# tomneda/DABstar

Measured on AMD Instinct MI355X. Metric: DAB Mode-I ensembles/s (2.048 MS/s IQ->MSC bytes) per GPU; FIB CRC match %, higher is better.
Workload: dtype f32+i32

## Files before the change

### dabstar_amd/csrc/deliver.hip

```cpp
#include "pipeline.h"
#include "packet_core.h"
#include "pad_core.h"
#include "mot_core.h"
#include "carousel_core.h"
#include "mp2_core.h"
#include "aac_core.h"
#include "eti_core.h"
#include "tii_core.h"
#include "scope_core.h"
#include "fig00.h"

namespace dabx {

__global__ __launch_bounds__(128) void k_deliver_front(EngineDev e, DeliverDev dv)
{
  const int s = blockIdx.x, tid = threadIdx.x;
  const StreamCtl &c = e.ctl[s];
  uint8_t *slab = dv.slab;
  if (s == 0 && tid == 0) *reinterpret_cast<dabx_chunk_header *>(slab) = dv.hdr;
  const int F = dv.hdr.max_frames;
  const long long done = dv.frames_done[s], have = c.frames - done;
  int n = (int)(have < F ? have : F);
  if (n > e.out_frames) n = e.out_frames;
  if (!(dv.hdr.what & DABX_DELIVER_FIB)) n = (int)(have < F ? have : F);
// ... 39 lines not shown
  if (pre) {
    const BatchSnap bs = e.snap[sj / e.max_subch];
    cif_out += msc_new_frames(bs.msc_done, bs.cif_no, sc.start_cif).n;
  }
  const int cap_cifs = 4 * dv.hdr.max_frames;
  const long long have = cif_out - dv.cif_done[sj];
  LfRange q;
  q.n = (int)(have < cap_cifs ? have : cap_cifs);
  if (q.n > MSC_SLOTS) q.n = MSC_SLOTS;
  if (q.n < 0) q.n = 0;
  q.lost = (int)(have > q.n ? have - q.n : 0);
  q.first = cif_out - q.n;
  const bool want_lf = (dv.hdr.what & DABX_DELIVER_MSC) || ((dv.hdr.what & DABX_DELIVER_MSC_NOT_DABPLUS) && !sc.dab_plus);
  if (!want_lf) { q.lost = 0; q.first = cif_out; q.n = 0; }
  return q;
}

__global__ __launch_bounds__(64) void k_deliver_lf(EngineDev e, DeliverDev dv)
{
  const int sj = blockIdx.x, lane = threadIdx.x;
  const SubchDev &sc = e.subch[sj];
  if (!(sc.active && e.msc_out && !e.fic_only)) return;
  const LfRange q = deliver_lf_range(e, dv, sj, sc, true);
  if (q.n == 0) return;
  const uint8_t *ring = e.msc_out + (size_t)sj * MSC_SLOTS * e.msc_stride;
  uint32_t *o = reinterpret_cast<uint32_t *>(dv.slab + dv.layout_off[3 * (size_t)sj]);
  const int wpf = 3 * sc.kbps / 4;
  for (int f = 0; f < q.n; f++) {
    const uint32_t *src = reinterpret_cast<const uint32_t *>(ring + (size_t)((q.first + f) % MSC_SLOTS) * e.msc_stride);
    for (int w = lane; w < wpf; w += 64) o[(size_t)f * wpf + w] = src[w];
  }
}

__global__ __launch_bounds__(64) void k_deliver_msc(EngineDev e, DeliverDev dv, int with_lf)
{
  const int sj = blockIdx.x, lane = threadIdx.x;
  const SubchDev &sc = e.subch[sj];
  uint8_t *slab = dv.slab;
  const unsigned long long msc_off = dv.layout_off[3 * (size_t)sj], sf_off = dv.layout_off[3 * (size_t)sj + 1], sfi_off = dv.layout_off[3 * (size_t)sj + 2];
  const int R = sc.kbps / 8, nb = 3 * sc.kbps, sfb = 110 * R, pitch = (sfb + 3) & ~3;
  const int cap_sf = (4 * dv.hdr.max_frames + 4) / 5;
  long long c_done = dv.cif_done[sj], s_done = dv.sf_done[sj];
  int n_c = 0, n_s = 0, lost_c = 0, lost_s = 0;
  long long first_c = c_done, first_s = s_done;
  const bool live = sc.active && e.msc_out && !e.fic_only;
  if (live) {
    const long long have_s = sc.sf_count - s_done;
    const LfRange q = deliver_lf_range(e, dv, sj, sc, false);
    n_c = q.n; lost_c = q.lost; first_c = q.first;
    n_s = (int)(have_s < cap_sf ? have_s : cap_sf);
    if (n_s > SF_SLOTS) n_s = SF_SLOTS;
    if (n_s < 0) n_s = 0;
    lost_s = (int)(have_s > n_s ? have_s - n_s : 0);
    first_s = sc.sf_count - n_s;
    if (with_lf && n_c) {
      const uint8_t *ring = e.msc_out + (size_t)sj * MSC_SLOTS * e.msc_stride;
      uint32_t *o = reinterpret_cast<uint32_t *>(slab + msc_off);
      const int wpf = nb / 4;
      for (int f = 0; f < n_c; f++) {
        const uint32_t *src = reinterpret_cast<const uint32_t *>(ring + (size_t)((first_c + f) % MSC_SLOTS) * e.msc_stride);
        for (int w = lane; w < wpf; w += 64) o[(size_t)f * wpf + w] = src[w];
      }
    }
    if ((dv.hdr.what & DABX_DELIVER_SF) && sc.dab_plus) {
      const uint8_t *ring = e.sf_out + (size_t)sj * SF_SLOTS * e.sf_stride;
      uint32_t *o = reinterpret_cast<uint32_t *>(slab + sf_off);
      const int wpf = pitch / 4;
      for (int f = 0; f < n_s; f++) {
        const uint32_t *src = reinterpret_cast<const uint32_t *>(ring + (size_t)((first_s + f) % SF_SLOTS) * e.sf_stride);
        for (int w = lane; w < wpf; w += 64) o[(size_t)f * wpf + w] = src[w];
      }
      if (e.sf_info && lane < 8 * n_s) {
        const uint32_t *inf = reinterpret_cast<const uint32_t *>(e.sf_info + (size_t)sj * SF_SLOTS);
        uint32_t *oi = reinterpret_cast<uint32_t *>(slab + sfi_off);
        for (int w = lane; w < 8 * n_s; w += 64) oi[w] = inf[(size_t)((first_s + (w >> 3)) % SF_SLOTS) * 8 + (w & 7)];
      }
    }
  }
  if (lane == 0) {
    dabx_chunk_subch r;
    r.active = live ? 1 : 0; r.subch_id = dv.subch_id[sj]; r.kbps = sc.kbps; r.dab_plus = sc.dab_plus;
    r.start_cif = sc.start_cif; r.first_cif = first_c; r.n_cifs = n_c; r.cifs_lost = lost_c;
    r.first_sf = first_s; r.n_sf = n_s; r.sf_lost = lost_s; r.msc_off = msc_off; r.sf_off = sf_off; r.sf_pitch = pitch; r.reserved = 0;
    r.sf_ok = sc.sf_ok; r.sf_fail = sc.sf_fail; r.rs_corrected = sc.rs_corr; r.rs_failed = sc.rs_fail; r.fc_corrected = sc.fc_corr;
    r.au_ok = sc.au_ok; r.au_bad = sc.au_bad; r.sfi_off = sfi_off;
    reinterpret_cast<dabx_chunk_subch *>(slab + dv.hdr.off_subch)[sj] = r;
    if (live) { dv.cif_done[sj] = sc.cif_out; dv.sf_done[sj] = sc.sf_count; }
  }
}

__global__ __launch_bounds__(64) void k_deliver_dg(PacketDev pk, uint8_t *slab, unsigned long long off_dg)
{
  PacketSlot &ps = pk.slots[blockIdx.x];
  if (!ps.out.dl_rec_off) return;
  const OutGather g = out_ring_gather(ps.out, slab, threadIdx.x);
  if (threadIdx.x == 0) {
    dabx_chunk_dg t;
// ... 183 lines not shown
}

__global__ __launch_bounds__(256) void k_deliver_scope(EngineDev e, ScopeDeliverDev sd)
{
  const int s = blockIdx.x, tid = threadIdx.x;
  constexpr int CAP = DABX_CHUNK_FRAMES < SCOPE_RING ? DABX_CHUNK_FRAMES : SCOPE_RING, SLOT_Q = SCOPE_SLOT_BYTES / 16;
  static_assert(SCOPE_SLOT_BYTES % 16 == 0, "a record slot is copied in 16-byte words");
  const unsigned long long rec_off = sd.rec_off[s];
  const long long total = sd.ring ? sd.shows[(size_t)s * sd.st_stride] : 0, have = rec_off ? total - sd.done[s] : 0;
  int n = (int)(have < CAP ? have : CAP);
  if (n < 0) n = 0;
  const long long first = total - n;
  if (tid == 0) {
    dabx_chunk_scope r;
    r.first_record = first; r.n_records = n; r.records_lost = (int)(have > n ? have - n : 0); r.rec_off = rec_off; r.records_total = total;
    reinterpret_cast<dabx_chunk_scope *>(sd.slab + sd.off_scope)[s] = r;
  }
  uint4 *o = reinterpret_cast<uint4 *>(sd.slab + rec_off);
  for (int i = tid; i < n * SLOT_Q; i += 256) {
    const int k = i / SLOT_Q, wd = i - k * SLOT_Q;
    o[i] = reinterpret_cast<const uint4 *>(sd.ring + ((size_t)s * SCOPE_RING + (size_t)((first + k) % SCOPE_RING)) * SCOPE_SLOT_BYTES)[wd];
  }
  __syncthreads();
  if (tid == 0) sd.done[s] = total;
}

int launch_deliver_scope(const EngineDev &e, const ScopeDeliverDev &sd, hipStream_t st)
{
  hipLaunchKernelGGL(k_deliver_scope, dim3(e.n_streams), dim3(256), 0, st, e, sd);
  DABX_HIP(hipGetLastError());
  return 0;
}

int launch_deliver_msc(const EngineDev &e, const DeliverDev &dv, hipStream_t st, bool with_lf)
{
  if (e.max_subch <= 0) return 0;
  hipLaunchKernelGGL(k_deliver_msc, dim3(e.n_streams * e.max_subch), dim3(64), 0, st, e, dv, with_lf ? 1 : 0);
  DABX_HIP(hipGetLastError());
  return 0;
}
int launch_deliver_lf(const EngineDev &e, const DeliverDev &dv, hipStream_t st)
{
  if (e.max_subch <= 0 || !dv.lf_done) return 0;
  hipLaunchKernelGGL(k_deliver_lf, dim3(e.n_streams * e.max_subch), dim3(64), 0, st, e, dv);
  DABX_HIP(hipEventRecord(dv.lf_done, st));
  DABX_HIP(hipGetLastError());
  return 0;
}

__global__ __launch_bounds__(128) void k_eti_front(EngineDev e, EtiDev t)
{
  constexpr int F = MSC_BATCH_FRAMES;
  __shared__ int32_t found[12 * F], fhi[12 * F], flo[12 * F];
  const int s = blockIdx.x, tid = threadIdx.x;
  const StreamCtl &c = e.ctl[s];
  const EtiFront cur = t.front[s];
  EtiStage &st = t.stage[s];
  const long long frames = c.frames, have = frames - cur.fib_frames;
  const int n = have < 0 ? 0 : (int)(have < F ? have : F);
  const long long first = frames - n;
  for (int i = tid; i < n * 96; i += 128) {
    const int f = i / 96, w = i - 96 * f;
    const size_t slot = (size_t)s * e.out_frames + (size_t)((first + f) % e.out_frames);
    st.fib[f][w] = reinterpret_cast<const uint32_t *>(e.fib_out + slot * 384)[w];
  }
  for (int q = tid; q < 12 * n; q += 128) {
    const int f = q / 12, i = q - 12 * f;
    const size_t slot = (size_t)s * e.out_frames + (size_t)((first + f) % e.out_frames);
    int hi = -1, lo = -1;
    found[q] = e.fib_crc[slot * 12 + i] && fib_fig00_counter(e.fib_out + slot * 384 + 32 * i, &hi, &lo);
// ... 207 lines not shown
```

### dabstar_amd/csrc/engine.h

```cpp
#pragma once
#include "pipeline.h"
#include "packet_core.h"
#include "pad_core.h"
#include "mot_core.h"
#include "carousel_core.h"
#include "mp2_core.h"
#include "aac_core.h"
#include "tii_core.h"
#include "scope_core.h"
#include "sdma.h"
#include "iqfile.h"
#include <algorithm>
#include <condition_variable>
#include <deque>
#include <mutex>
#include <string>
#include <thread>
#include <vector>

using namespace dabx;

static constexpr int DL_FRAMES = MSC_BATCH_FRAMES;

struct Delivery {
  bool open = false;
  int what = 0;
  int copy_engine = 0;
  static constexpr int NDEV = 3;
  uint8_t *dev[NDEV] = {nullptr, nullptr, nullptr};
  hipEvent_t packed[NDEV] = {nullptr, nullptr, nullptr};
  hipEvent_t packed_lf[NDEV] = {nullptr, nullptr, nullptr};
  bool dev_busy[NDEV] = {false, false, false};
  hipStream_t cs = nullptr;
  Sdma sdma;
  size_t capacity = 0, bytes = 0;
  enum { FREE = 0, IN_FLIGHT = 1, LANDED = 2, HELD = 3 };
  struct Slot { uint8_t *host = nullptr; uint64_t sig = 0, sig2 = 0; int state = FREE; uint64_t seq = 0; size_t bytes = 0, lf_from = 0; int devslab = 0; };
  std::vector<Slot> slots;
  std::deque<int> queue;
  std::deque<int> jobs;
  std::mutex mu;
  std::condition_variable cv;
  std::thread copier;
  bool quit = false;
  int device = 0;
  std::string copier_error;
  uint64_t next_seq = 0, landed = 0, bytes_copied = 0;
  double copy_s = 0, copy_s_max = 0, gather_wait_s = 0, calib_gbps = 0;
  unsigned long long *layout_off = nullptr;
  int32_t *subch_id = nullptr;
  long long *frames_done = nullptr, *cif_done = nullptr, *sf_done = nullptr;
  dabx_chunk_header hdr{};
  bool want_pad = false;
  bool want_mot = false;
  bool want_dg = false;
  EtiFront *eti_front = nullptr;
  long long *eti_next = nullptr;
  EtiStage *eti_stage[NDEV] = {nullptr, nullptr, nullptr};
  size_t eti_rows_off = 0;
  dabx_chunk_header_ext ext{};
  long long *tii_done = nullptr;
  long long *scope_done = nullptr;
  unsigned long long *scope_off = nullptr;
  std::vector<char> scope_room;
  bool scope() const { return (what & DABX_DELIVER_SCOPE) != 0; }
  bool tii() const { return (what & DABX_DELIVER_TII) != 0; }
  bool mp2_audio() const { return (what & DABX_DELIVER_MP2_AUDIO) != 0; }
  bool aac() const { return (what & DABX_DELIVER_AAC) != 0; }
  bool eti() const { return (what & DABX_DELIVER_ETI) != 0; }
  EtiDev eti_dev(int devslab) const
  {
    return EtiDev{eti_front, eti_next, eti_stage[devslab], dev[devslab], subch_id, hdr.off_eti, eti_rows_off, hdr.max_frames, 0};
  }
};

struct Ingest {
  bool open = false;
  int copy_engine = 0, max_frames = 0;
  size_t capacity = 0;
  struct Slab {
    uint8_t *host = nullptr, *dev = nullptr; uint64_t sig = 0; bool in_flight = false;
    size_t bytes = 0, pitch = 0;
    std::vector<size_t> n_bytes;
    IqJob *jobs_host = nullptr, *jobs_dev = nullptr;
// ... 179 lines not shown
```

### dabstar_amd/csrc/engine_delivery.cpp

```cpp
#include "engine.h"
#include <algorithm>
#include <chrono>
#include <cstddef>
#include <cstring>
#include <string>
#include <thread>
#include <vector>

static_assert(sizeof(dabx_chunk_header) == 128 && sizeof(dabx_chunk_stream) == 72 && sizeof(dabx_chunk_frame) == 16 && sizeof(dabx_chunk_subch) == 144 && offsetof(dabx_chunk_header, off_mot) == 112 &&
              sizeof(dabx_superframe_info) == 32 && sizeof(dabx_chunk_eti) == 64 && offsetof(dabx_chunk_header, off_eti) == 120 &&
              sizeof(dabx_chunk_header_ext) == 64 && sizeof(dabx_chunk_tii) == 32 && sizeof(dabx_tii_event) == 32 && sizeof(dabx_tii_result) == 16 &&
              sizeof(dabx_chunk_mp2_audio) == 128 && offsetof(dabx_chunk_header_ext, off_mp2_audio) == 16 &&
              sizeof(dabx_chunk_aac) == 128 && offsetof(dabx_chunk_header_ext, off_aac) == 24,
              "include/dabx.h: chunk record layout");
static constexpr int DL_SF_CAP = (4 * DL_FRAMES + 4) / 5;
#if DABX_MSC_BATCH == 7
static_assert(DL_FRAMES == DABX_CHUNK_FRAMES, "include/dabx.h: DABX_CHUNK_FRAMES is the library's MSC batch");
#endif

template <class Tab> static size_t layout_section(Tab &tab, bool want, size_t off, size_t table_bytes, uint64_t *off_table)
{
  bool any = false;
  for (auto &q : tab.host) { q.st.out.dl_rec_off = q.st.out.dl_bytes_off = 0; any = any || q.on; }
  if (!want || !any) return off;
// ... 97 lines not shown

int dabx_engine::delivery_begin(DeliverDev *dv, int *slot, int *devslab)
{
  Delivery &D = dl;
  int h = -1;
  uint64_t seq;
  {
    std::unique_lock<std::mutex> lk(D.mu);
    if (!D.copier_error.empty()) { set_error("delivery: %s", D.copier_error.c_str()); return DABX_E_HIP; }
    for (size_t i = 0; i < D.slots.size() && h < 0; i++) if (D.slots[i].state == Delivery::FREE) h = (int)i;
    if (h < 0) { set_error("delivery: no free host slab (dabx_delivery_release)"); return DABX_E_STATE; }
    seq = D.next_seq++;
    const int k = (int)(seq % Delivery::NDEV);
    if (!D.cv.wait_for(lk, std::chrono::seconds(30), [&]() { return !D.dev_busy[k] || !D.copier_error.empty(); })) {
      D.next_seq--;
      set_error("delivery: device slab %d still busy after 30 s (chunk %llu)", k, (unsigned long long)seq);
      return DABX_E_STATE;
    }
    if (!D.copier_error.empty()) { D.next_seq--; set_error("delivery: %s", D.copier_error.c_str()); return DABX_E_HIP; }
    D.dev_busy[k] = true;
    D.slots[(size_t)h].state = Delivery::IN_FLIGHT;
    D.slots[(size_t)h].seq = seq;
    D.slots[(size_t)h].devslab = k;
    *devslab = k;
  }
  dv->slab = D.dev[*devslab]; dv->layout_off = D.layout_off; dv->subch_id = D.subch_id;
  dv->frames_done = D.frames_done; dv->cif_done = D.cif_done; dv->sf_done = D.sf_done;
  dv->hdr = D.hdr; dv->hdr.seq = seq;
  dv->off_mp2_audio = D.ext.off_mp2_audio;
  dv->off_aac = D.ext.off_aac;
  const size_t lf_from = (size_t)D.hdr.off_msc;
  const bool split = D.copy_engine == 0 && D.bytes > lf_from && D.bytes - lf_from >= ((size_t)1 << 20) && !dev.fic_only && dev.max_subch > 0 && dev.msc_out;
  dv->lf_done = split ? D.packed_lf[*devslab] : nullptr;
  {
    std::lock_guard<std::mutex> lk(D.mu);
    D.slots[(size_t)h].lf_from = split ? lf_from : 0;
  }
  *slot = h;
  int rc = launch_deliver_front(dev, *dv, stream);
  if (!rc && D.eti()) rc = launch_eti_front(dev, D.eti_dev(*devslab), stream, mk);
  if (!rc && D.tii())
    rc = launch_deliver_tii(dev, TiiDeliverDev{D.dev[*devslab], D.ext, D.tii_done, tiis.dev.ring, tiis.exists() ? &tiis.dev.cnt->events : nullptr,
                                               (int32_t)(sizeof(TiiCounters) / sizeof(long long)), 0}, stream);
  else if (!rc && D.ext.magic) rc = launch_deliver_ext(D.ext, D.dev[*devslab], stream);
  if (!rc && D.scope())
    rc = launch_deliver_scope(dev, ScopeDeliverDev{D.dev[*devslab], D.ext.off_scope, D.scope_off, D.scope_done, scope.dev.ring,
                                                   scope.exists() ? &scope.dev.st->shows : nullptr, (int32_t)(sizeof(ScopeState) / sizeof(long long)), 0}, stream);
  if (rc) {
    std::lock_guard<std::mutex> lk(D.mu);
    D.dev_busy[*devslab] = false;
    D.slots[(size_t)h].state = Delivery::FREE;
    D.next_seq--;
    D.cv.notify_all();
  }
  return rc;
}

void dabx_engine::delivery_abort(int slot, int devslab)
{
  Delivery &D = dl;
  std::lock_guard<std::mutex> lk(D.mu);
  D.slots[(size_t)slot].state = Delivery::FREE;
  D.dev_busy[devslab] = false;
  if (D.next_seq > 0) D.next_seq--;
  if (D.copier_error.empty()) D.copier_error = "a chunk was abandoned after a failed launch: " + std::string(dabx::last_error());
  D.cv.notify_all();
}

int dabx_engine::delivery_finish(int slot, int devslab, hipStream_t tail)
{
  Delivery &D = dl;
  {
    const hipError_t he = hipEventRecord(D.packed[devslab], tail);
    if (he != hipSuccess) {
      set_error("HIP error %d (%s) at %s:%d", (int)he, hipGetErrorString(he), __FILE__, __LINE__);
      delivery_abort(slot, devslab);
      return DABX_E_HIP;
    }
  }
  std::lock_guard<std::mutex> lk(D.mu);
  D.slots[(size_t)slot].bytes = D.bytes;
  D.queue.push_back(slot);
  D.jobs.push_back(slot);
  D.cv.notify_all();
  return 0;
// ... 65 lines not shown
  return 0;
}

void delivery_free(dabx_engine *e)
{
  Delivery &D = e->dl;
  if (D.copier.joinable()) {
    { std::lock_guard<std::mutex> lk(D.mu); D.quit = true; D.cv.notify_all(); }
    D.copier.join();
  }
  D.quit = false;
  if (D.cs) (void)hipStreamSynchronize(D.cs);
  for (auto &sl : D.slots) { if (sl.host) (void)hipHostFree(sl.host); sdma_signal_destroy(sl.sig); sdma_signal_destroy(sl.sig2); }
  D.slots.clear();
  D.queue.clear();
  D.jobs.clear();
  for (int k = 0; k < Delivery::NDEV; k++) {
    if (D.dev[k]) (void)hipFree(D.dev[k]);
    if (D.packed[k]) (void)hipEventDestroy(D.packed[k]);
    if (D.packed_lf[k]) (void)hipEventDestroy(D.packed_lf[k]);
    D.dev[k] = nullptr; D.packed[k] = nullptr; D.packed_lf[k] = nullptr; D.dev_busy[k] = false;
  }
  for (void *q : {(void *)D.layout_off, (void *)D.subch_id, (void *)D.frames_done, (void *)D.cif_done, (void *)D.sf_done, (void *)D.eti_front,
                  (void *)D.eti_next, (void *)D.eti_stage[0], (void *)D.eti_stage[1], (void *)D.eti_stage[2], (void *)D.tii_done, (void *)D.scope_done,
                  (void *)D.scope_off}) if (q) (void)hipFree(q);
  D.tii_done = nullptr; D.ext = dabx_chunk_header_ext{};
  D.scope_done = nullptr; D.scope_off = nullptr; D.scope_room.clear();
  D.layout_off = nullptr; D.subch_id = nullptr; D.frames_done = D.cif_done = D.sf_done = nullptr;
  D.eti_front = nullptr; D.eti_next = nullptr; D.eti_rows_off = 0;
  for (int k = 0; k < Delivery::NDEV; k++) D.eti_stage[k] = nullptr;
  if (D.cs) (void)hipStreamDestroy(D.cs);
  D.cs = nullptr;
  D.copier_error.clear();
  D.open = false; D.capacity = D.bytes = 0; D.next_seq = 0;
  D.landed = D.bytes_copied = 0; D.copy_s = D.copy_s_max = D.gather_wait_s = 0;
}

}

extern "C" {

int dabx_delivery_open(dabx_engine *e, const dabx_delivery_config *cfg)
{
  if (!e || (cfg && (cfg->host_slabs < 0 || cfg->host_slabs == 1 || cfg->host_slabs > 64 || (cfg->what & ~(1023 | DABX_DELIVER_AAC | DABX_DELIVER_SCOPE)) || cfg->copy_engine < 0 || cfg->copy_engine > 1))) {
    set_error("dabx_delivery_open: bad argument");
    return DABX_E_ARG;
  }
  if (cfg && cfg->what == DABX_DELIVER_TII) {
    set_error("dabx_delivery_open: DABX_DELIVER_TII needs at least one other DABX_DELIVER_* bit beside it");
    return DABX_E_ARG;
  }
  if (cfg && (cfg->what & DABX_DELIVER_MP2_AUDIO) && !(cfg->what & ~(DABX_DELIVER_MP2_AUDIO | DABX_DELIVER_TII))) {
    set_error("dabx_delivery_open: DABX_DELIVER_MP2_AUDIO needs at least one DABX_DELIVER_* bit below 256 beside it");
    return DABX_E_ARG;
  }
  if (cfg && (cfg->what & DABX_DELIVER_AAC) && !(cfg->what & ~(DABX_DELIVER_AAC | DABX_DELIVER_MP2_AUDIO | DABX_DELIVER_TII))) {
    set_error("dabx_delivery_open: DABX_DELIVER_AAC needs at least one DABX_DELIVER_* bit below 256 beside it");
    return DABX_E_ARG;
  }
  if (cfg && (cfg->what & DABX_DELIVER_SCOPE) &&
      !(cfg->what & ~(DABX_DELIVER_SCOPE | DABX_DELIVER_AAC | DABX_DELIVER_MP2_AUDIO | DABX_DELIVER_TII | DABX_DELIVER_ETI))) {
    set_error("dabx_delivery_open: DABX_DELIVER_SCOPE needs at least one DABX_DELIVER_* bit below 128 beside it");
    return DABX_E_ARG;
  }
  if (e->dl.open) { set_error("dabx_delivery_open: already open"); return DABX_E_STATE; }
  int rc = sync_all(e);
  if (rc) return rc;
// ... 193 lines not shown
```

### dabstar_amd/csrc/engine_facade.cpp

```cpp
#include "engine.h"
#include "viterbi_core.h"
#include <cstring>
#include <vector>

static int fic_engine_create(int batch, dabx_engine **out)
{
  auto *e = *out = new dabx_engine();
  (void)hipGetDevice(&e->device);
  if (hipStreamCreateWithFlags(&e->stream, hipStreamNonBlocking) != hipSuccess) { delete e; *out = nullptr; return DABX_E_HIP; }
  e->ss.a = e->stream;
  EngineDev &d = e->dev;
  d.n_streams = batch; d.max_subch = 0; d.out_frames = 1; d.fic_only = 1;
  d.vit_stride = (int)vit_scratch_words(FIC_OUT);
  int rc;
  if ((rc = e->alloc(&d.ctl, batch)) || (rc = e->alloc(&d.fic_sym, (size_t)batch * 3 * K2)) || (rc = e->alloc(&d.fib_out, (size_t)batch * 384)) ||
      (rc = e->alloc(&d.fib_crc, (size_t)batch * 12)) || (rc = e->alloc(&d.vit_scratch, (size_t)batch * 4 * d.vit_stride, false))) return rc;
  std::vector<StreamCtl> ctl(batch);
  for (auto &c : ctl) { memset(&c, 0, sizeof(c)); c.frame_ok = 1; }
  DABX_HIP(hipMemcpyAsync(d.ctl, ctl.data(), sizeof(StreamCtl) * batch, hipMemcpyHostToDevice, e->stream));
  DABX_HIP(hipStreamSynchronize(e->stream));
  return 0;
}

extern "C" {
// ... 422 lines not shown
  m->slots[(size_t)slot] = dabx_subch_desc{};
  return msc_apply(m);
}

int dabx_msc_stop_all_services(dabx_msc *m)
{
  if (!m) return DABX_E_ARG;
  for (auto &s : m->slots) s = dabx_subch_desc{};
  return msc_apply(m);
}

int dabx_msc_is_service_running(dabx_msc *m, int slot)
{
  if (!m || slot < 0 || slot >= (int)m->slots.size()) return DABX_E_ARG;
  return m->slots[(size_t)slot].kbps != 0;
}

int dabx_msc_process_block(dabx_msc *m, const int16_t *soft, int blk_nr)
{
  if (!m || !soft || blk_nr < 4 || blk_nr >= L) { set_error("dabx_msc_process_block: bad argument"); return DABX_E_ARG; }
  dabx_engine *e = m->eng;
  if (int rc = use_device(e)) return rc;
  if (e->classes_dirty) {
    if (int rc = e->build_msc_classes()) return rc;
    e->classes_dirty = false;
  }
  const int cur = (blk_nr - 4) % 18;
  const bool closes = cur == 17;
  DABX_HIP(hipMemcpyAsync(m->soft_dev, soft, sizeof(int16_t) * K2, hipMemcpyHostToDevice, e->stream));
  int rc = launch_stage_msc_block(e->dev, m->soft_dev, cur, closes, e->stream);
  if (rc) return rc;
  if (!closes) { DABX_HIP(hipStreamSynchronize(e->stream)); return 0; }
  e->dev.snap = e->snap_buf[e->ss.batch_parity];
  if ((rc = launch_msc_batch(e->dev, 1, nullptr, e->ss, e->mk))) return rc;
  if ((rc = sync_all(e))) return rc;
  std::vector<SubchDev> sc(m->slots.size());
  DABX_HIP(hipMemcpy(sc.data(), e->dev.subch, sizeof(SubchDev) * sc.size(), hipMemcpyDeviceToHost));
  for (size_t j = 0; j < sc.size(); j++) {
    m->frames_seen[j] = m->frames_now[j]; m->sf_seen[j] = m->sf_now[j];
    m->frames_now[j] = sc[j].active ? sc[j].cif_out : 0;
    m->sf_now[j] = sc[j].active ? sc[j].sf_count : 0;
  }
  return 1;
}

int dabx_msc_get_frame(dabx_msc *m, int slot, uint8_t *bytes, int max_bytes)
{
  if (!m || slot < 0 || slot >= (int)m->slots.size() || !bytes) return DABX_E_ARG;
  const size_t j = (size_t)slot;
  if (!m->slots[j].kbps || m->frames_now[j] == m->frames_seen[j]) return 0;
  const int nb = 3 * m->slots[j].kbps;
  if (max_bytes < nb) { set_error("dabx_msc_get_frame: %d bytes needed", nb); return DABX_E_ARG; }
  const int got = dabx_read_msc(m->eng, 0, slot, 1, bytes);
  return got < 0 ? got : (got == 1 ? nb : 0);
}

int dabx_msc_get_superframe(dabx_msc *m, int slot, uint8_t *bytes, int max_bytes)
{
  if (!m || slot < 0 || slot >= (int)m->slots.size() || !bytes) return DABX_E_ARG;
  const size_t j = (size_t)slot;
  if (!m->slots[j].kbps || m->sf_now[j] == m->sf_seen[j]) return 0;
  const int nb = 110 * m->slots[j].kbps / 8;
  if (max_bytes < nb) { set_error("dabx_msc_get_superframe: %d bytes needed", nb); return DABX_E_ARG; }
  const int got = dabx_read_superframes(m->eng, 0, slot, 1, bytes);
  return got < 0 ? got : (got == 1 ? nb : 0);
}
// ... 18 lines not shown
```

### dabstar_amd/csrc/msc_stages.hip

```cpp
#include "pipeline.h"
#include "packet_core.h"
#include "pad_core.h"
#include "mot_core.h"
#include "carousel_core.h"
#include "mp2_core.h"
#include "aac_core.h"
#include "fec_core.h"
#include "wave_ops.h"

namespace dabx {

__global__ __launch_bounds__(64, 4) void k_dabplus(EngineDev e, DevTables t)
{
  const int job = blockIdx.x, lane = threadIdx.x;
  const int s = job / e.max_subch, j = job % e.max_subch;
  SubchDev &sc = e.subch[(size_t)s * e.max_subch + j];
  if (!sc.active) return;
  const BatchSnap bs = e.snap[s];
  const long long n_new = msc_new_frames(bs.msc_done, bs.cif_no, sc.start_cif).n;
  if (n_new == 0) return;
  const int R = sc.kbps / 8, nbytes = 3 * sc.kbps;
  const uint8_t *ring = e.msc_out + ((size_t)s * e.max_subch + j) * MSC_SLOTS * e.msc_stride;
  long long cif_out = sc.cif_out;
  int blocks_in_buf = sc.blocks_in_buf, sf_sync = sc.sf_sync;
// ... 149 lines not shown
        case 2: n_au = 6; s_au[0] = 11; s_au[1] = hdr[3] * 16 + (hdr[4] >> 4); s_au[2] = (hdr[4] & 0xf) * 256 + hdr[5];
                s_au[3] = hdr[6] * 16 + (hdr[7] >> 4); s_au[4] = (hdr[7] & 0xf) * 256 + hdr[8];
                s_au[5] = hdr[9] * 16 + (hdr[10] >> 4); s_au[6] = end; break;
        default: n_au = 3; s_au[0] = 6; s_au[1] = hdr[3] * 16 + (hdr[4] >> 4); s_au[2] = (hdr[4] & 0xf) * 256 + hdr[5];
                s_au[3] = end; break;
        }
        s_au[7] = n_au;
      }
      s_flag = flag;
    }
    __syncthreads();
    const int flag = s_flag;
    if (flag & 1) {
      if (flag & 2) fc_corr++;
      sf_sync = 4; sf_ok++;
      const int n_au = s_au[7];
      int good = 0, bad = 0;
      unsigned crc_mask = 0, len_mask = 0;
      for (int a = 0; a < n_au; a++) {
        const int st = s_au[a], len = s_au[a + 1] - st - 2;
        if (len > 960 || len < 0 || st + len + 2 > 110 * R) { bad++; len_mask |= 1u << a; continue; }
        const int per = (len + 63) >> 6, from = lane * per, to = min(len, from + per);
        const unsigned xp_slice = s_xpow[from < to ? len - to : 0];
        const unsigned first2 = len >= 2 ? 0xFFu : 0u;
        unsigned crc = 0;
        for (int i = from; i < to; i++) crc = (s_crc[(win[st + i] ^ (i < 2 ? first2 : 0u) ^ (crc >> 8)) & 0xFF] ^ (crc << 8)) & 0xFFFFu;
        unsigned acc = from < to ? crc_mulmod(crc, xp_slice) : 0u;
        if (len < 2 && lane == 0) acc ^= crc_mulmod(0xFFFFu, s_xpow[len]);
        acc = wave_xor(acc);
        const unsigned want = ((unsigned)win[st + len] << 8) | win[st + len + 1];
        if (((~acc) & 0xFFFFu) == want) { good++; crc_mask |= 1u << a; } else bad++;
      }
      au_ok += good; au_bad += bad;
      if (lane == 0 && e.sf_info) {
        dabx_superframe_info r;
        r.num_aus = (uint8_t)n_au; r.au_crc_ok = (uint8_t)crc_mask; r.au_len_bad = (uint8_t)len_mask; r.stream_parms = (uint8_t)(win[2] & 0x7F);
#pragma unroll
        for (int a = 0; a < 7; a++) r.au_start[a] = a <= n_au ? (uint16_t)s_au[a] : (uint16_t)0;
        r.rs_corrected = (uint16_t)corr; r.rs_failed = (uint8_t)fail; r.fc_corrected = (flag & 2) ? 1 : 0; r.reserved = 0;
        r.first_frame = oldest;
        e.sf_info[((size_t)s * e.max_subch + j) * SF_SLOTS + (size_t)(sf_count % SF_SLOTS)] = r;
      }
      uint8_t *sfo = e.sf_out + (((size_t)s * e.max_subch + j) * SF_SLOTS + (size_t)(sf_count % SF_SLOTS)) * e.sf_stride;
      for (int i = lane; i < (110 * R + 3) / 4; i += 64)
        reinterpret_cast<uint32_t *>(sfo)[i] = reinterpret_cast<const uint32_t *>(win)[i];
      sf_count++;
    } else {
      sf_sync--;
      if (sf_sync == 0) { blocks_in_buf = 4; sf_fail++; }
    }
  }
  if (lane == 0) {
    sc.cif_out = cif_out; sc.blocks_in_buf = blocks_in_buf; sc.sf_sync = sf_sync; sc.sf_count = sf_count;
    sc.sf_ok += sf_ok; sc.sf_fail += sf_fail; sc.rs_corr += rs_corr; sc.rs_fail += rs_fail;
    sc.fc_corr += fc_corr; sc.au_ok += au_ok; sc.au_bad += au_bad;
  }
}

__global__ __launch_bounds__(64) void k_packet(PacketDev pk)
{
  const int lane = threadIdx.x;
  PacketSlot &ps = pk.slots[blockIdx.x];
  const SubchDev &sc = pk.subch[(size_t)ps.s * pk.max_subch + ps.j];
  if (!sc.active) return;
  const BatchSnap bs = pk.snap[ps.s];
  const long long n_new = msc_new_frames(bs.msc_done, bs.cif_no, sc.start_cif).n;
  if (n_new == 0) return;
  const int nbytes = 3 * sc.kbps, n_gran = sc.kbps / 8;
  const uint8_t *ring = pk.msc_out + ((size_t)ps.s * pk.max_subch + ps.j) * MSC_SLOTS * pk.msc_stride;
  __shared__ __attribute__((aligned(16))) uint8_t frm[3 * PKT_MAX_KBPS];
  __shared__ uint16_t s_crc[256], s_xpow[128];
  __shared__ unsigned s_info[64];
  __shared__ uint16_t s_part[64];
  for (int i = lane; i < 256; i += 64) s_crc[i] = pk.crc_ccitt[i];
  for (int i = lane; i < 128; i += 64) s_xpow[i] = pk.crc_xpow[i];
  const int address = ps.address;
  uint8_t *const dg_ring = ps.out.bytes;
  dabx_datagroup_info *const dg_recs = ps.out.recs;
// ... 602 lines not shown
```

### dabstar_amd/csrc/pipeline.h

```cpp
#pragma once
#include "dabx_internal.h"
#include "ring_fmt.h"

namespace dabx {

#ifndef DABX_MSC_BATCH
#define DABX_MSC_BATCH 7
#endif
constexpr int MSC_SLOTS = DABX_MSC_BATCH > 7 ? 64 : 32;
constexpr int MSC_BATCH_FRAMES = DABX_MSC_BATCH;
constexpr int SF_SLOTS = 16;
constexpr int ACQ_NEED = 20 * TU + 50 + (TF + 1) + (TN + 50 + 21) + 64;
constexpr int FRAME_NEED = TF + 2 * TU;
constexpr int FEW_STREAMS = 48;

enum StreamState : int32_t { ST_INIT = 0, ST_WAIT_SYNC = 1, ST_EVAL_SYNC = 2 };

struct StreamCtl {
  unsigned long long rd;
  unsigned long long sym0_pos;
  long long cif_no;
  long long msc_done_cif;
  long long frames;
  int32_t state;
// ... 23 lines not shown
  float lvl_anchor_S;
  int32_t pad3_;
  long long lvl_rewalks, lvl_unanchored;
  long long lvl_healed;
  unsigned long long lvl_hist_pos[16];
  float lvl_hist_S[16];
};
constexpr int LVL_HIST = 16;

struct SubchDev {
  int32_t cu_start, cu_size, kbps, prot_level, short_form, dab_plus;
  int32_t nbits;
  int32_t active;
  int32_t fast_class, pad_;
  const uint16_t *map;
  long long start_cif;
  long long cif_out;
  int32_t blocks_in_buf, sf_sync;
  long long sf_count;
  long long sf_ok, sf_fail, rs_corr, rs_fail, fc_corr, au_ok, au_bad;
  long long move_cif;
  int32_t prev_cu_start, pad2_;
};
#ifdef __HIPCC__
__device__ __forceinline__ int msc_move_thr(const SubchDev &sc, long long r)
{
  const long long t = sc.move_cif - r + 16;
  return t <= 0 ? 0 : (t >= 16 ? 16 : (int)t);
}
#endif

struct BatchSnap { long long msc_done, cif_no; };
struct FrameSnap { long long cif0; float clock_err; int32_t frame_ok, np_sel, pad_; };

struct EngineDev {
  int32_t n_streams, max_subch, out_frames;
  int32_t ring_len;
  float threshold;
  int32_t strongest, fic_only, capture_soft;
  int32_t exact_level;
  int32_t anchor_level;
  unsigned long long *wr_horizon;
  unsigned long long *level_pos;
  int32_t *locked_count;
  int32_t tie_mode;
  int32_t msc_stride;
  int32_t sf_stride;
  int32_t vit_stride;
  void *iq;
  int32_t ring_fmt;
  unsigned long long *wr;
  StreamCtl *ctl;
  DemapDev demap;
  float2 *spectra;
  FrameSnap *fsnap;
  int32_t *demap_busy;
  float *dciq_state;
  unsigned long long *dciq_done;
  int32_t parity;
  int32_t s0;
  int32_t flag_sync;
  uint32_t step_seq;
  uint32_t *sym_seq, *fic_seq;
  int32_t *seq_timeouts;
  double2 *nco_tid;
  double2 *nco_sym;
  int32_t *sym_off;
  float2 *cp_part;
  float *abs_part;
  uint8_t *fic_sym;
  uint8_t *tdi;
  uint32_t *vit_scratch;
  SubchDev *subch;
  uint8_t *fib_out;
  uint8_t *fib_crc;
  long long *frame_pos;
  int32_t *frame_start;
  uint8_t *msc_out;
  uint8_t *sf_out;
  dabx_superframe_info *sf_info;
  int16_t *soft_cap;
  BatchSnap *snap;
  float2 *tii_acc;
  int32_t *tii_cnt;
};

struct DeliverDev {
  uint8_t *slab;
  const unsigned long long *layout_off;
  const int32_t *subch_id;
  long long *frames_done;
  long long *cif_done, *sf_done;
  dabx_chunk_header hdr;
  unsigned long long off_mp2_audio;
  unsigned long long off_aac;
  hipEvent_t lf_done;
};

struct EtiFront { long long fib_frames; int32_t hi, lo; };
struct EtiStage {
  long long first_frame, hi_cif;
  int32_t n_frames, end_hi, end_lo, pad_;
  int32_t hi[MSC_BATCH_FRAMES], lo[MSC_BATCH_FRAMES];
  uint32_t fib[MSC_BATCH_FRAMES][96];
  long long fib_frames;
};
struct EtiDev {
  EtiFront *front;
  long long *next_cif;
  EtiStage *stage;
  uint8_t *slab;
  const int32_t *subch_id;
  unsigned long long off_eti, rows_off;
  int32_t max_frames, pad_;
};

struct TiiDeliverDev {
  uint8_t *slab;
  dabx_chunk_header_ext ext;
  long long *done;
  const uint8_t *ring;
  const long long *events;
  int32_t cnt_stride, pad_;
};

struct ScopeDeliverDev {
  uint8_t *slab;
  unsigned long long off_scope;
  const unsigned long long *rec_off;
// ... 137 lines not shown
{
  return (size_t)(cif & (TDI_SLOTS - 1)) * CIF_BITS + (size_t)(i & 15) * (CIF_BITS / 16) + (size_t)(i >> 4);
}
#endif

struct PacketDev;
struct PadDev;
struct MotDev;
struct CarouselDev;
struct Mp2AudioDev;
struct AacStreamDev;
struct ScopeDev;
extern const char *const kStepKernelNames[N_STEP_KERNELS];
int launch_front_step(const EngineDev &e, EngineStreams &ss, Marker &mk, bool async_acquire, bool all_locked, const ScopeDev *scope = nullptr);
int launch_msc_batch(const EngineDev &e, int cifs, const MscFast *fast, EngineStreams &ss, Marker &mk, const DeliverDev *dv = nullptr,
                     hipStream_t *tail = nullptr, const PacketDev *pk = nullptr, const PadDev *pad = nullptr, const MotDev *mot = nullptr,
                     const CarouselDev *car = nullptr, const EtiDev *eti = nullptr, const Mp2AudioDev *mp2a = nullptr, long long *mp2a_launches = nullptr,
                     const AacStreamDev *aac = nullptr, long long *aac_launches = nullptr);
int launch_dciq(const EngineDev &e, int mode, hipStream_t st);
int launch_level_exact(const EngineDev &e, hipStream_t st);
int launch_commit(const EngineDev &e, int stream, unsigned long long n, hipStream_t st);
int launch_fic_only(const EngineDev &e, hipStream_t st, int first, int count);
int launch_i16_to_sym(const int16_t *soft, uint8_t *sym, size_t n, hipStream_t st);
int launch_stage_msc_block(const EngineDev &e, const int16_t *soft_dev, int blk, bool closes_cif, hipStream_t st);
int launch_msc_inject(const EngineDev &e, int stream, const int16_t *soft_dev, int n_cifs, int first, hipStream_t st);
int launch_msc_advance(const EngineDev &e, const int32_t *counts_dev, hipStream_t st);
int launch_fic_inject(const EngineDev &e, int stream, const int16_t *soft_dev, hipStream_t st);
int launch_fic_decode(const EngineDev &e, const int32_t *present_dev, hipStream_t st);
int launch_demap_inject(const EngineDev &e, int parity, int stream, const float2 *spec_dev, const float2 *null_dev, float clock_err, int np_sel, hipStream_t st);
int launch_demap_frame(const EngineDev &e, unsigned step_count, const int32_t *present_dev, int schedule, hipStream_t st, const ScopeDev *scope = nullptr);
int launch_msc_prep(const EngineDev &e, int cifs, const MscLaunch &L, hipStream_t st, Marker &mk);
int launch_msc_vitT(const EngineDev &e, int cifs, const MscLaunch &L, hipStream_t st, Marker &mk);
int launch_deliver_front(const EngineDev &e, const DeliverDev &dv, hipStream_t st);
int launch_deliver_msc(const EngineDev &e, const DeliverDev &dv, hipStream_t st, bool with_lf);
int launch_deliver_lf(const EngineDev &e, const DeliverDev &dv, hipStream_t st);
int launch_deliver_dg(const EngineDev &e, const DeliverDev &dv, const PacketDev &pk, hipStream_t st);
int launch_deliver_pad(const EngineDev &e, const DeliverDev &dv, const PadDev &pd, hipStream_t st);
int launch_deliver_mot(const EngineDev &e, const DeliverDev &dv, const MotDev &md, hipStream_t st);
int launch_deliver_carousel(const EngineDev &e, const DeliverDev &dv, const CarouselDev &cd, hipStream_t st, bool clear_table);
int launch_deliver_mp2_audio(const EngineDev &e, const DeliverDev &dv, const Mp2AudioDev &ad, unsigned long long off_mp2_audio, hipStream_t st);
int launch_deliver_aac(const EngineDev &e, const DeliverDev &dv, const AacStreamDev &ad, unsigned long long off_aac, hipStream_t st);
int launch_deliver_ext(const dabx_chunk_header_ext &ext, uint8_t *slab, hipStream_t st);
int launch_deliver_tii(const EngineDev &e, const TiiDeliverDev &td, hipStream_t st);
int launch_deliver_scope(const EngineDev &e, const ScopeDeliverDev &sd, hipStream_t st);
int launch_eti_front(const EngineDev &e, const EtiDev &t, hipStream_t st, Marker &mk);
int launch_eti_back(const EngineDev &e, const EtiDev &t, hipStream_t st, Marker &mk, bool pre);
int launch_dabplus_stage(const EngineDev &e, hipStream_t st, Marker &mk);
int launch_packet_stage(const EngineDev &e, const PacketDev *pk, hipStream_t st, Marker &mk, PacketDev *used);
int launch_pad_stage(const EngineDev &e, const PadDev *pad, hipStream_t st, Marker &mk, PadDev *used);
int launch_mot_stage(const EngineDev &e, const MotDev *mot, const PadDev &pad, hipStream_t st, Marker &mk, MotDev *used);
int launch_mp2_audio_stage(const EngineDev &e, const Mp2AudioDev *ma, hipStream_t st, Mp2AudioDev *used);
int launch_aac_stream_stage(const EngineDev &e, const AacStreamDev *aa, hipStream_t st, AacStreamDev *used);
int launch_carousel_stage(const EngineDev &e, const CarouselDev *car, const PacketDev &pk, hipStream_t st, Marker &mk, CarouselDev *used);
void dabx_internal_fibdec_skip(dabx_fibdec *d, long long n_fibs);

}
```

### dabstar_amd/csrc/pipeline.hip

```cpp
#include <type_traits>
#include "pipeline.h"
#include "packet_core.h"
#include "pad_core.h"
#include "mot_core.h"
#include "carousel_core.h"
#include "mp2_core.h"
#include "aac_core.h"
#include <algorithm>
#include "ofdm_core.h"
#include "scope_core.h"
#include "viterbi_core.h"
#include "fec_core.h"
#include "acq_walk.h"
#include "level_par.h"
#include "fig00.h"

namespace dabx {

__device__ __forceinline__ void front_prio() { __builtin_amdgcn_s_setprio(3); }

template <class T> __device__ __forceinline__ T uniform_load(const T *p)
{
  typedef unsigned Raw __attribute__((ext_vector_type(sizeof(T) / 4)));
  const Raw raw = *(const __attribute__((address_space(4))) Raw *)(const void *)p;
// ... 1595 lines not shown
  } while (0)
  auto demap = [&](hipStream_t q, int l0, int l1) {
    DABX_DEMAP_DISPATCH(k_demap_frame6, dim3(e.n_streams), dim3(DEMAP_THREADS), 0, q, e, *t, l0, l1);
  };
  if (ss.d && ss.fic_on_d) {
    hipLaunchKernelGGL(k_sym_publish, dim3((e.n_streams + 63) / 64), dim3(64), 0, st, e);
    if ((rc = launch_scope(e, *t, scope, ss.d))) return rc;
    mk.begin(3, ss.d);
    DABX_DEMAP_DISPATCH(k_demap_whole, dim3(e.n_streams), dim3(DEMAP_THREADS), 0, ss.d, e, *t);
    mk.end(3, ss.d);
    ss.demap_in_flight = true; ss.demap_unrecorded = true;
  } else if (ss.d) {
    if (ss.demap_in_flight) { DABX_HIP(hipStreamWaitEvent(st, ss.demap_done, 0)); ss.demap_in_flight = false; }
    if ((rc = launch_scope(e, *t, scope, st))) return rc;
    mk.begin(10, st);
    DABX_DEMAP_DISPATCH(k_demap_fic, dim3(e.n_streams), dim3(DEMAP_THREADS), 0, st, e, *t);
    mk.end(10, st);
    DABX_HIP(hipEventRecord(ss.fic_go, st));
    DABX_HIP(hipStreamWaitEvent(ss.d, ss.fic_go, 0));
    mk.begin(3, ss.d); demap(ss.d, 3, 75); mk.end(3, ss.d);
    DABX_HIP(hipEventRecord(ss.demap_done, ss.d));
    ss.demap_in_flight = true;
  } else {
    if ((rc = launch_scope(e, *t, scope, st))) return rc;
    mk.begin(3, st); demap(st, 0, 75); mk.end(3, st);
  }
  mk.begin(4, st); hipLaunchKernelGGL(k_fic_frame, dim3(e.n_streams), dim3(256), 0, st, e, *t, 0, 4); mk.end(4, st);
  mk.begin(5, st); DABX_LAUNCH_RING(e, k_frame_tail, dim3(e.n_streams), dim3(256), 0, st, e, *t); mk.end(5, st);
  if (e.exact_level && ss.tail_done) { DABX_HIP(hipEventRecord(ss.tail_done, st)); ss.tail_recorded = true; }
  DABX_HIP(hipGetLastError());
  return 0;
}

int launch_msc_batch(const EngineDev &e, int cifs, const MscFast *fast, EngineStreams &ss, Marker &mk, const DeliverDev *dv, hipStream_t *tail,
                     const PacketDev *pk, const PadDev *pad, const MotDev *mot, const CarouselDev *car, const EtiDev *eti, const Mp2AudioDev *mp2a,
                     long long *mp2a_launches, const AacStreamDev *aac, long long *aac_launches)
{
  const DevTables *t;
  int rc = get_tables(&t);
  if (rc) return rc;
  if (tail) *tail = ss.a;
  if (e.fic_only || e.max_subch <= 0 || !e.msc_out) {
    if (dv && (rc = launch_deliver_msc(e, *dv, ss.a, true))) return rc;
    if (dv && eti && (rc = launch_eti_back(e, *eti, ss.a, mk, false))) return rc;
    return 0;
  }
  const int jobs = e.n_streams * cifs * e.max_subch;
  auto wait_for_demapper = [&](hipStream_t who) -> int {
    if (!ss.demap_in_flight) return 0;
    if (ss.demap_unrecorded) { DABX_HIP(hipEventRecord(ss.demap_done, ss.d)); ss.demap_unrecorded = false; }
    DABX_HIP(hipStreamWaitEvent(who, ss.demap_done, 0));
    if (who == ss.a) ss.demap_in_flight = false;
    return 0;
  };
  if (ss.msc_in_flight) { DABX_HIP(hipStreamWaitEvent(ss.a, ss.msc_done, 0)); ss.msc_in_flight = false; }
  hipLaunchKernelGGL(k_msc_snap, dim3((e.n_streams + 255) / 256), dim3(256), 0, ss.a, e, cifs);
  MscLaunch L{};
  unsigned fast_mask = 0;
  long long fast_jobs = 0, fast_pairs = 0;
  if (fast) {
    for (int c = 0; c < fast->n_cls; c++) fast_jobs += (long long)fast->cls[c].n_pairs * cifs;
    if (fast_jobs >= fast->min_jobs)
      for (int c = 0; c < fast->n_cls; c++) {
        const MscClass &k = fast->cls[c];
        MscLaunchCls &o = L.c[L.n++];
        o.n_in = k.n_in; o.nbits = k.nbits; o.n_pairs = k.n_pairs; o.g0 = L.groups;
        o.map2 = k.map2; o.pairs = k.pairs; o.inT = k.inT[ss.batch_parity]; o.decT = k.decT;
        L.groups += (int)(((long long)k.n_pairs * cifs + 63) / 64);
        fast_mask |= 1u << c;
        fast_pairs += k.n_pairs;
      }
  }
  hipStream_t sb = ss.b ? ss.b : ss.a;
  if (ss.b) {
    DABX_HIP(hipEventRecord(ss.prep_done, ss.a));
    DABX_HIP(hipStreamWaitEvent(ss.b, ss.prep_done, 0));
// ... 13 lines not shown
      mk.end(8, ss.a);
      if (ss.b) {
        DABX_HIP(hipEventRecord(ss.prep_done, ss.a));
        DABX_HIP(hipStreamWaitEvent(ss.b, ss.prep_done, 0));
      }
    }
  } else {
    if ((rc = wait_for_demapper(sb))) return rc;
    mk.begin(8, sb);
    hipLaunchKernelGGL(k_msc_frame, dim3((jobs + 3) / 4), dim3(256), 0, sb, e, *t, cifs, 0u);
    mk.end(8, sb);
    if (ss.b) {
      DABX_HIP(hipEventRecord(ss.prep_b_done, ss.b));
      ss.prep_pending = true;
    }
  }
  if (dv && eti && dv->lf_done && (rc = launch_eti_back(e, *eti, sb, mk, true))) return rc;
  if (dv && (rc = launch_deliver_lf(e, *dv, sb))) return rc;
  PacketDev p;
  PadDev q;
  MotDev m;
  CarouselDev c;
  Mp2AudioDev au;
  AacStreamDev ac;
  if ((rc = launch_packet_stage(e, pk, sb, mk, &p))) return rc;
  if ((rc = launch_carousel_stage(e, car, p, sb, mk, &c))) return rc;
  if ((rc = launch_dabplus_stage(e, sb, mk))) return rc;
  if ((rc = launch_pad_stage(e, pad, sb, mk, &q))) return rc;
  if ((rc = launch_mot_stage(e, mot, q, sb, mk, &m))) return rc;
  if ((rc = launch_mp2_audio_stage(e, mp2a, sb, &au))) return rc;
  if (au.n > 0 && mp2a_launches) ++*mp2a_launches;
  if ((rc = launch_aac_stream_stage(e, aac, sb, &ac))) return rc;
  if (ac.n > 0 && aac_launches) ++*aac_launches;
  if (dv && (rc = launch_deliver_msc(e, *dv, sb, !dv->lf_done))) return rc;
  if (dv && eti && !dv->lf_done && (rc = launch_eti_back(e, *eti, sb, mk, false))) return rc;
  if (dv && p.n > 0 && (rc = launch_deliver_dg(e, *dv, p, sb))) return rc;
  if (dv && q.n > 0 && (rc = launch_deliver_pad(e, *dv, q, sb))) return rc;
  if (dv && m.n > 0 && (rc = launch_deliver_mot(e, *dv, m, sb))) return rc;
  if (dv && c.n > 0 && (rc = launch_deliver_carousel(e, *dv, c, sb, m.n <= 0))) return rc;
  if (dv && au.n > 0 && (rc = launch_deliver_mp2_audio(e, *dv, au, dv->off_mp2_audio, sb))) return rc;
  if (dv && ac.n > 0 && (rc = launch_deliver_aac(e, *dv, ac, dv->off_aac, sb))) return rc;
  if (tail) *tail = sb;
  if (ss.b) {
    DABX_HIP(hipEventRecord(ss.msc_done, ss.b));
    ss.msc_in_flight = true;
  }
  ss.batch_parity ^= 1;
  DABX_HIP(hipGetLastError());
  return 0;
}

int launch_fic_only(const EngineDev &e, hipStream_t st, int first, int count)
{
  const DevTables *t;
  int rc = get_tables(&t);
  if (rc) return rc;
  hipLaunchKernelGGL(k_fic_frame, dim3(e.n_streams), dim3(256), 0, st, e, *t, first, count);
  DABX_HIP(hipGetLastError());
  return 0;
}

__global__ void k_i16_to_sym(const int16_t *soft, uint8_t *sym, size_t n)
{
  const size_t i = (size_t)blockIdx.x * blockDim.x + threadIdx.x;
  if (i < n) sym[i] = soft_to_sym(soft[i]);
}
int launch_i16_to_sym(const int16_t *soft, uint8_t *sym, size_t n, hipStream_t st)
// ... 148 lines not shown
```

Before: 550,900.

## Write DAB+ superframes directly into delivery slab from the producer kernel

When no backlog exists, the superframe stage writes each superframe and its info record straight into the delivery slab as well as the ring. The deliver_msc kernel then skips the superframe ring-to-slab copy, and when no copies remain it runs one thread per subchannel instead of one 64-lane block each. The aim is to remove a redundant device-memory pass and shrink the metadata-only launch. A backlog flag falls back to the old copy path after FIC-closing batches, which adds state tracking and a risk of mismatched slab positions.

Result: no change. 549,900 (-0.2%).

```diff
diff --git a/dabstar_amd/csrc/deliver.hip b/dabstar_amd/csrc/deliver.hip
--- a/dabstar_amd/csrc/deliver.hip
+++ b/dabstar_amd/csrc/deliver.hip
@@ -95,9 +95,11 @@
   }
 }
 
-__global__ __launch_bounds__(64) void k_deliver_msc(EngineDev e, DeliverDev dv, int with_lf)
-{
-  const int sj = blockIdx.x, lane = threadIdx.x;
+__global__ __launch_bounds__(64) void k_deliver_msc(EngineDev e, DeliverDev dv, int with_lf, int with_sf)
+{
+  const bool copies = with_lf || with_sf;
+  const int sj = copies ? (int)blockIdx.x : (int)(blockIdx.x * 64 + threadIdx.x), lane = copies ? (int)threadIdx.x : 0;
+  if (sj >= e.n_streams * e.max_subch) return;
   const SubchDev &sc = e.subch[sj];
   uint8_t *slab = dv.slab;
   const unsigned long long msc_off = dv.layout_off[3 * (size_t)sj], sf_off = dv.layout_off[3 * (size_t)sj + 1], sfi_off = dv.layout_off[3 * (size_t)sj + 2];
@@ -125,7 +127,7 @@
         for (int w = lane; w < wpf; w += 64) o[(size_t)f * wpf + w] = src[w];
       }
     }
-    if ((dv.hdr.what & DABX_DELIVER_SF) && sc.dab_plus) {
+    if (with_sf && (dv.hdr.what & DABX_DELIVER_SF) && sc.dab_plus) {
       const uint8_t *ring = e.sf_out + (size_t)sj * SF_SLOTS * e.sf_stride;
       uint32_t *o = reinterpret_cast<uint32_t *>(slab + sf_off);
       const int wpf = pitch / 4;
@@ -375,10 +377,11 @@
   return 0;
 }
 
-int launch_deliver_msc(const EngineDev &e, const DeliverDev &dv, hipStream_t st, bool with_lf)
+int launch_deliver_msc(const EngineDev &e, const DeliverDev &dv, hipStream_t st, bool with_lf, bool with_sf)
 {
   if (e.max_subch <= 0) return 0;
-  hipLaunchKernelGGL(k_deliver_msc, dim3(e.n_streams * e.max_subch), dim3(64), 0, st, e, dv, with_lf ? 1 : 0);
+  const int slots = e.n_streams * e.max_subch;
+  hipLaunchKernelGGL(k_deliver_msc, dim3(with_lf || with_sf ? slots : (slots + 63) / 64), dim3(64), 0, st, e, dv, with_lf ? 1 : 0, with_sf ? 1 : 0);
   DABX_HIP(hipGetLastError());
   return 0;
 }
diff --git a/dabstar_amd/csrc/engine.h b/dabstar_amd/csrc/engine.h
--- a/dabstar_amd/csrc/engine.h
+++ b/dabstar_amd/csrc/engine.h
@@ -50,6 +50,7 @@
   unsigned long long *layout_off = nullptr;
   int32_t *subch_id = nullptr;
   long long *frames_done = nullptr, *cif_done = nullptr, *sf_done = nullptr;
+  bool backlog = false;
   dabx_chunk_header hdr{};
   bool want_pad = false;
   bool want_mot = false;
diff --git a/dabstar_amd/csrc/engine_delivery.cpp b/dabstar_amd/csrc/engine_delivery.cpp
--- a/dabstar_amd/csrc/engine_delivery.cpp
+++ b/dabstar_amd/csrc/engine_delivery.cpp
@@ -153,6 +153,9 @@
   const size_t lf_from = (size_t)D.hdr.off_msc;
   const bool split = D.copy_engine == 0 && D.bytes > lf_from && D.bytes - lf_from >= ((size_t)1 << 20) && !dev.fic_only && dev.max_subch > 0 && dev.msc_out;
   dv->lf_done = split ? D.packed_lf[*devslab] : nullptr;
+  const bool had_backlog = D.backlog;
+  dv->direct = !had_backlog;
+  D.backlog = false;
   {
     std::lock_guard<std::mutex> lk(D.mu);
     D.slots[(size_t)h].lf_from = split ? lf_from : 0;
@@ -172,6 +175,7 @@
     D.dev_busy[*devslab] = false;
     D.slots[(size_t)h].state = Delivery::FREE;
     D.next_seq--;
+    D.backlog = had_backlog;
     D.cv.notify_all();
   }
   return rc;
@@ -303,7 +307,7 @@
   if (D.cs) (void)hipStreamDestroy(D.cs);
   D.cs = nullptr;
   D.copier_error.clear();
-  D.open = false; D.capacity = D.bytes = 0; D.next_seq = 0;
+  D.open = false; D.capacity = D.bytes = 0; D.next_seq = 0; D.backlog = false;
   D.landed = D.bytes_copied = 0; D.copy_s = D.copy_s_max = D.gather_wait_s = 0;
 }
 
diff --git a/dabstar_amd/csrc/engine_facade.cpp b/dabstar_amd/csrc/engine_facade.cpp
--- a/dabstar_amd/csrc/engine_facade.cpp
+++ b/dabstar_amd/csrc/engine_facade.cpp
@@ -478,6 +478,7 @@
   if (rc) return rc;
   if (!closes) { DABX_HIP(hipStreamSynchronize(e->stream)); return 0; }
   e->dev.snap = e->snap_buf[e->ss.batch_parity];
+  if (e->dl.open) e->dl.backlog = true;
   if ((rc = launch_msc_batch(e->dev, 1, nullptr, e->ss, e->mk))) return rc;
   if ((rc = sync_all(e))) return rc;
   std::vector<SubchDev> sc(m->slots.size());
diff --git a/dabstar_amd/csrc/msc_stages.hip b/dabstar_amd/csrc/msc_stages.hip
--- a/dabstar_amd/csrc/msc_stages.hip
+++ b/dabstar_amd/csrc/msc_stages.hip
@@ -205,6 +205,17 @@
         if (((~acc) & 0xFFFFu) == want) { good++; crc_mask |= 1u << a; } else bad++;
       }
       au_ok += good; au_bad += bad;
+      uint32_t *sf2 = nullptr;
+      dabx_superframe_info *sfi2 = nullptr;
+      if (e.direct.slab) {
+        const size_t sj = (size_t)s * e.max_subch + j;
+        const unsigned long long sf_off = e.direct.layout_off[3 * sj + 1], sfi_off = e.direct.layout_off[3 * sj + 2];
+        const long long pos = sf_count - sc.sf_count;
+        if (sf_off && pos < e.direct.sf_cap) {
+          sf2 = reinterpret_cast<uint32_t *>(e.direct.slab + sf_off + (size_t)pos * (size_t)((110 * R + 3) & ~3));
+          if (sfi_off) sfi2 = reinterpret_cast<dabx_superframe_info *>(e.direct.slab + sfi_off) + pos;
+        }
+      }
       if (lane == 0 && e.sf_info) {
         dabx_superframe_info r;
         r.num_aus = (uint8_t)n_au; r.au_crc_ok = (uint8_t)crc_mask; r.au_len_bad = (uint8_t)len_mask; r.stream_parms = (uint8_t)(win[2] & 0x7F);
@@ -213,10 +224,14 @@
         r.rs_corrected = (uint16_t)corr; r.rs_failed = (uint8_t)fail; r.fc_corrected = (flag & 2) ? 1 : 0; r.reserved = 0;
         r.first_frame = oldest;
         e.sf_info[((size_t)s * e.max_subch + j) * SF_SLOTS + (size_t)(sf_count % SF_SLOTS)] = r;
+        if (sfi2) *sfi2 = r;
       }
       uint8_t *sfo = e.sf_out + (((size_t)s * e.max_subch + j) * SF_SLOTS + (size_t)(sf_count % SF_SLOTS)) * e.sf_stride;
-      for (int i = lane; i < (110 * R + 3) / 4; i += 64)
-        reinterpret_cast<uint32_t *>(sfo)[i] = reinterpret_cast<const uint32_t *>(win)[i];
+      for (int i = lane; i < (110 * R + 3) / 4; i += 64) {
+        const uint32_t v = reinterpret_cast<const uint32_t *>(win)[i];
+        reinterpret_cast<uint32_t *>(sfo)[i] = v;
+        if (sf2) sf2[i] = v;
+      }
       sf_count++;
     } else {
       sf_sync--;
diff --git a/dabstar_amd/csrc/pipeline.h b/dabstar_amd/csrc/pipeline.h
--- a/dabstar_amd/csrc/pipeline.h
+++ b/dabstar_amd/csrc/pipeline.h
@@ -79,6 +79,11 @@
 
 struct BatchSnap { long long msc_done, cif_no; };
 struct FrameSnap { long long cif0; float clock_err; int32_t frame_ok, np_sel, pad_; };
+struct DirectDev {
+  uint8_t *slab;
+  const unsigned long long *layout_off;
+  int32_t sf_cap, pad_;
+};
 
 struct EngineDev {
   int32_t n_streams, max_subch, out_frames;
@@ -130,6 +135,7 @@
   BatchSnap *snap;
   float2 *tii_acc;
   int32_t *tii_cnt;
+  DirectDev direct;
 };
 
 struct DeliverDev {
@@ -142,6 +148,7 @@
   unsigned long long off_mp2_audio;
   unsigned long long off_aac;
   hipEvent_t lf_done;
+  bool direct;
 };
 
 struct EtiFront { long long fib_frames; int32_t hi, lo; };
@@ -345,7 +352,7 @@
 int launch_msc_prep(const EngineDev &e, int cifs, const MscLaunch &L, hipStream_t st, Marker &mk);
 int launch_msc_vitT(const EngineDev &e, int cifs, const MscLaunch &L, hipStream_t st, Marker &mk);
 int launch_deliver_front(const EngineDev &e, const DeliverDev &dv, hipStream_t st);
-int launch_deliver_msc(const EngineDev &e, const DeliverDev &dv, hipStream_t st, bool with_lf);
+int launch_deliver_msc(const EngineDev &e, const DeliverDev &dv, hipStream_t st, bool with_lf, bool with_sf);
 int launch_deliver_lf(const EngineDev &e, const DeliverDev &dv, hipStream_t st);
 int launch_deliver_dg(const EngineDev &e, const DeliverDev &dv, const PacketDev &pk, hipStream_t st);
 int launch_deliver_pad(const EngineDev &e, const DeliverDev &dv, const PadDev &pd, hipStream_t st);
diff --git a/dabstar_amd/csrc/pipeline.hip b/dabstar_amd/csrc/pipeline.hip
--- a/dabstar_amd/csrc/pipeline.hip
+++ b/dabstar_amd/csrc/pipeline.hip
@@ -1651,7 +1651,7 @@
   return 0;
 }
 
-int launch_msc_batch(const EngineDev &e, int cifs, const MscFast *fast, EngineStreams &ss, Marker &mk, const DeliverDev *dv, hipStream_t *tail,
+int launch_msc_batch(const EngineDev &e_in, int cifs, const MscFast *fast, EngineStreams &ss, Marker &mk, const DeliverDev *dv, hipStream_t *tail,
                      const PacketDev *pk, const PadDev *pad, const MotDev *mot, const CarouselDev *car, const EtiDev *eti, const Mp2AudioDev *mp2a,
                      long long *mp2a_launches, const AacStreamDev *aac, long long *aac_launches)
 {
@@ -1659,8 +1659,14 @@
   int rc = get_tables(&t);
   if (rc) return rc;
   if (tail) *tail = ss.a;
+  const bool direct = dv && dv->direct;
+  EngineDev e = e_in;
+  if (direct) {
+    const int cap_sf = (4 * dv->hdr.max_frames + 4) / 5;
+    e.direct = DirectDev{dv->slab, dv->layout_off, cap_sf < SF_SLOTS ? cap_sf : SF_SLOTS, 0};
+  }
   if (e.fic_only || e.max_subch <= 0 || !e.msc_out) {
-    if (dv && (rc = launch_deliver_msc(e, *dv, ss.a, true))) return rc;
+    if (dv && (rc = launch_deliver_msc(e, *dv, ss.a, true, true))) return rc;
     if (dv && eti && (rc = launch_eti_back(e, *eti, ss.a, mk, false))) return rc;
     return 0;
   }
@@ -1740,7 +1746,7 @@
   if (au.n > 0 && mp2a_launches) ++*mp2a_launches;
   if ((rc = launch_aac_stream_stage(e, aac, sb, &ac))) return rc;
   if (ac.n > 0 && aac_launches) ++*aac_launches;
-  if (dv && (rc = launch_deliver_msc(e, *dv, sb, !dv->lf_done))) return rc;
+  if (dv && (rc = launch_deliver_msc(e, *dv, sb, !dv->lf_done, !direct))) return rc;
   if (dv && eti && !dv->lf_done && (rc = launch_eti_back(e, *eti, sb, mk, false))) return rc;
   if (dv && p.n > 0 && (rc = launch_deliver_dg(e, *dv, p, sb))) return rc;
   if (dv && q.n > 0 && (rc = launch_deliver_pad(e, *dv, q, sb))) return rc;
```
